# s22s/erased-cells

Hardware: AMD Instinct MI355X
Metric: Gcells/s + HBM-GB/s roofline %, u8/u16->f64 16384^2, 1/2/4/8 GPUs (higher is better)
Workload: dtype f64

## Files before the change

### erased-cells_amd/csrc/ec_abi.hip

```cpp
#include <hip/hip_runtime.h>


#include <cfloat>
#include <cstdarg>
#include <cstdio>
#include <cstring>
#include <map>
#include <mutex>
#include <string>

#include "ec_lattice.hpp"
#include "ec_map_kernels.hpp"
#include "ec_reduce_kernels.hpp"
#include "ec_runtime.hpp"

namespace ecd {

static_assert(kMaxReduceBlocks <= kFinalizeMaxParts, "the finalize kernels read at most kFinalizeMaxParts partials");

static ec_status ensure_init() { return ensure_ready(); }

static int64_t* result_words(const Scratch& sc) { return sc.host_dev ? sc.host_dev : sc.dev_result(); }
static ec_status fetch_result(const Scratch& sc, int words, hipStream_t s) {
    if (!sc.host_dev) {
// ... 12 lines not shown
    }
    return nb < want ? nb : want;
}

static int reduce_cap(int per_cu) {
    const int knob = tuning().reduce_bpc;
    const long cap = long(device_cus()) * (knob > 0 ? knob : per_cu);
    return static_cast<int>(cap < kMaxReduceBlocks ? cap : kMaxReduceBlocks);
}

static inline hipStream_t S(ec_stream s) { return static_cast<hipStream_t>(s); }

template <typename Fn> struct pure_store : std::false_type {};
template <typename W> struct pure_store<FillFn<W>> : std::true_type {};

template <typename Fn, int U>
static void launch_map_u(const Fn& fn, size_t n, hipStream_t s) {
    const size_t groups = n / Fn::CPL;
    const size_t tiles = (groups + size_t(kBlock) * U - 1) / (size_t(kBlock) * U);
    const size_t stream_bytes[2] = {n * Fn::kIn0, n * Fn::kIn1};
    const unsigned lds = (pure_store<Fn>::value ? static_cast<unsigned>(tuning().write_lds_kb.load())
                                                : (Fn::kIn0 != 0 ? static_cast<unsigned>(tuning().map_lds_kb.load()) : 0u)) << 10;
    k_map<Fn, U><<<grid_for(tiles), kBlock, lds, s>>>(fn, n, cache_plan(stream_bytes, 2));
}

template <typename Fn>
static ec_status launch_map(const Fn& fn, size_t n, bool aligned, hipStream_t s, const char* what) {
    if (n == 0) return EC_OK;
    if (!aligned) {
        k_map_cellwise<Fn><<<grid_capped((n + kBlock - 1) / kBlock, 8), kBlock, 0, s>>>(fn, n);
    } else {
        switch (tuning().map_u) {
            case 1: launch_map_u<Fn, 1>(fn, n, s); break;
            case 4: launch_map_u<Fn, 4>(fn, n, s); break;
            default: launch_map_u<Fn, 2>(fn, n, s); break;
        }
    }
    return check_launch(what);
// ... 43 lines not shown
        const bool al = aligned16(p, p, p) && (!mask || aligned_to(mask, 16 / sizeof(T)));
        const int cap = reduce_cap(8);
        if (al) {
            const unsigned head = reduce_head(p, sizeof(T), n);
            const size_t groups = (n - head) / (16 / sizeof(T));
            auto launch = [&](auto u_tag, auto block_tag, int per_cu) {
                constexpr int U = decltype(u_tag)::value, BLOCK = decltype(block_tag)::value;
                static const int resident[2] = {resident_per_cu(k_min_max_partials<T, false, U, BLOCK>, BLOCK, per_cu),
                                                resident_per_cu(k_min_max_partials<T, true, U, BLOCK>, BLOCK, per_cu)};
                const int cap2 = reduce_cap(resident[mask ? 1 : 0]);
                size_t tiles = (groups + size_t(BLOCK) * U - 1) / (size_t(BLOCK) * U);
                if (tiles < 1) tiles = 1;
                grid = static_cast<unsigned>(tiles < size_t(cap2) ? tiles : size_t(cap2));
                int64_t* direct = grid == 1 ? keys2_dev : nullptr;
                const size_t stream_bytes[2] = {n * sizeof(T), mask ? n : 0};
                const unsigned hp = head | (cache_plan(stream_bytes, 2) << 8);
                if (mask) k_min_max_partials<T, true, U, BLOCK><<<grid, BLOCK, 0, s>>>(tp, mask, n, sc.dev, hp, direct);
                else k_min_max_partials<T, false, U, BLOCK><<<grid, BLOCK, 0, s>>>(tp, nullptr, n, sc.dev, hp, direct);
                return direct != nullptr;
            };
            using std::integral_constant;
            bool direct = false;
            switch (tuning().reduce_shape) {
                case 1: direct = launch(integral_constant<int, 16>{}, integral_constant<int, 512>{}, 4); break;
                case 2: direct = launch(integral_constant<int, 8>{}, integral_constant<int, 256>{}, 8); break;
                case 3: direct = launch(integral_constant<int, 8>{}, integral_constant<int, 1024>{}, 2); break;
                case 4: direct = launch(integral_constant<int, 4>{}, integral_constant<int, 512>{}, 4); break;
                default: direct = launch(integral_constant<int, kReduceU>{}, integral_constant<int, kRBlock>{}, 4); break;
            }
            if (direct) return check_launch("min_max(single workgroup)");
        } else {
// ... 244 lines not shown
    if (st != EC_OK) return st;
    st = fetch_result(sc, 2, S(stream));
    if (st != EC_OK) return st;
    return ec_min_max_decode(t, sc.host, mn, mx);
}

template <typename W>
static ec_status first_diff_w(const void* l, const void* r, size_t n, const Scratch& sc, hipStream_t s, unsigned* grid_out) {
    const int cap = reduce_cap(4);
    const bool al = aligned16(l, r, r);
    const unsigned head = al ? reduce_head(l, sizeof(W), n) : 0u;
    size_t tiles = al ? ((n - head) / (16 / sizeof(W)) + size_t(kRBlock) * kReduceU - 1) / (size_t(kRBlock) * kReduceU) : (n + kRBlock - 1) / kRBlock;
    if (tiles < 1) tiles = 1;
    const unsigned grid = static_cast<unsigned>(tiles < size_t(cap) ? tiles : size_t(cap));
    const size_t stream_bytes[2] = {n * sizeof(W), n * sizeof(W)};
    k_first_diff_partials<W, kReduceU><<<grid, kRBlock, 0, s>>>(static_cast<const W*>(l), static_cast<const W*>(r), n,
                                                               reinterpret_cast<uint64_t*>(sc.dev), al, head | (cache_plan(stream_bytes, 2) << 8));
    *grid_out = grid;
    return check_launch("first_diff(partials)");
}

extern "C" ec_status ec_first_difference(ec_dtype t, const void* l, const void* r, size_t n, uint64_t* index, ec_stream stream) {
    EC_REQUIRE_INIT();
    if (!ecl::valid(t)) return set_error(EC_ERR_UNSUPPORTED_TYPE, "ec_first_difference: bad dtype %d", int(t));
    if (!index || (n > 0 && (!l || !r))) return set_error(EC_ERR_ARG, "ec_first_difference: null pointer");
    *index = n;
    if (n == 0) return EC_OK;
    Scratch sc;
    ec_status st = get_scratch(S(stream), &sc);
    if (st != EC_OK) return st;
    std::lock_guard<std::mutex> turn(*sc.mu);
    unsigned grid = 0;
// ... 125 lines not shown
    Scratch sc;
    ec_status st = get_scratch(S(stream), &sc);
    if (st != EC_OK) return st;
    unsigned grid = 0;
    if (n > 0) {
        const int cap = reduce_cap(4);
        const bool al = aligned_to(m, 16);
        const unsigned head = al ? reduce_head(m, 1, n) : 0u;
        size_t tiles = al ? ((n - head) / 16 + size_t(kRBlock) * kReduceU - 1) / (size_t(kRBlock) * kReduceU) : (n + kRBlock - 1) / kRBlock;
        if (tiles < 1) tiles = 1;
        grid = static_cast<unsigned>(tiles < size_t(cap) ? tiles : size_t(cap));
        uint64_t* direct = grid == 1 ? counts2_dev : nullptr;
        const int one = tuning().counts_one_launch.load();
        uint64_t* acc = (!direct && ((one == 1 && n < (size_t(1) << 29)) || (one >= 2 && n < (size_t(1) << 40)))) ? reinterpret_cast<uint64_t*>(sc.dev_acc()) : nullptr;
        const size_t stream_bytes[1] = {n};
        k_mask_count_partials<kReduceU><<<grid, kRBlock, 0, S(stream)>>>(m, n, reinterpret_cast<uint64_t*>(sc.dev), al,
                                                                        head | (cache_plan(stream_bytes, 1) << 8), direct, acc, counts2_dev);
        st = check_launch("mask_counts(partials)");
        if (st != EC_OK || direct || acc) return st;
    }
    k_mask_count_finalize<<<1, kFinalizeBlock, 0, S(stream)>>>(reinterpret_cast<const uint64_t*>(sc.dev), static_cast<int>(grid), n, counts2_dev);
    return check_launch("mask_counts(finalize)");
}

extern "C" ec_status ec_mask_counts(const uint8_t* m, size_t n, uint64_t* n_true, uint64_t* n_false, ec_stream stream) {
    EC_REQUIRE_INIT();
    if (!n_true || !n_false) return set_error(EC_ERR_ARG, "ec_mask_counts: null pointer");
    Scratch sc;
    ec_status st = get_scratch(S(stream), &sc);
    if (st != EC_OK) return st;
    std::lock_guard<std::mutex> turn(*sc.mu);
    st = ec_mask_counts_device(m, n, reinterpret_cast<uint64_t*>(result_words(sc)), stream);
// ... 38 lines not shown
```

### erased-cells_amd/csrc/ec_binop_tu.hpp

```cpp
#pragma once

#include <hip/hip_runtime.h>

#include <cmath>

#include "ec_binop_kernels.hpp"
#include "ec_runtime.hpp"

namespace ecd {

static inline unsigned lds_cap(int knob, int rule_kb) { return static_cast<unsigned>(knob >= 0 ? knob : rule_kb) << 10; }

template <typename L, typename R, int OP>
static ec_status launch_binop_pair(const void* l, const void* r, size_t n, double* out, hipStream_t s) {
    const Tuning& tu = tuning();
    const L* lp = static_cast<const L*>(l);
    const R* rp = static_cast<const R*>(r);
    constexpr int U = kBinopU;
    if (!aligned16(l, r, out)) {
        k_binop_cellwise<L, R, OP><<<grid_capped((n + kBlock - 1) / kBlock, 8), kBlock, 0, s>>>(lp, rp, out, n);
        return check_launch("binop(cellwise)");
    }
    constexpr bool kCanStage = Staged<L>::value || Staged<R>::value;
    const int variant = tu.binop_variant.load();
    const size_t stream_bytes[2] = {n * sizeof(L), l == r ? 0 : n * sizeof(R)};
    unsigned policy = cache_plan(stream_bytes, 2, n * sizeof(double));
    if (l == r && (policy & 1u)) policy |= 2u;
    constexpr bool kRulePair = kCanStage && ((sizeof(L) == 8) != (sizeof(R) == 8)) && (sizeof(L) <= 4 || sizeof(R) <= 4);
    const bool by_rule = variant < 0 && kRulePair && policy == 0 && n >= (size_t(1) << 20);
    if (kCanStage && (variant == 1 || by_rule)) {
        const size_t tiles = (n / kLdsWaveCells + kWavesPerBlock - 1) / kWavesPerBlock;
        constexpr unsigned kStatic = kWavesPerBlock * unsigned(Staged<L>::kSlabBytes + Staged<R>::kSlabBytes);
        const int knob = tu.binop_lds_kb.load();
        const unsigned lds = knob >= 0 ? unsigned(knob) << 10 : by_rule ? 32000u - kStatic : 0u;
        k_binop_lds<L, R, OP, kNtStore, kNtLoad><<<grid_for(tiles), kBlock, lds, s>>>(lp, rp, out, n);
        if (by_rule) lds_rule_launches().fetch_add(1, std::memory_order_relaxed);
        return check_launch(by_rule ? "binop(lds, by rule)" : "binop(lds)");
    }
    const LoadedStream st[2] = {{l, sizeof(L)}, {r, sizeof(R)}};
    const unsigned head = peel_head(st, 2, n);
    const size_t tiles = (((n - head) >> 1) + size_t(kBlock) * U - 1) / (size_t(kBlock) * U);
    k_binop_direct<L, R, OP, U, kNtStore, kNtLoad><<<grid_for(tiles), kBlock, lds_cap(tuning().binop_lds_kb.load(), sizeof(L) == 8 && sizeof(R) == 8 ? 48 : 0), s>>>(lp, rp, out, n, head | (policy << 8));
    return check_launch("binop(direct)");
}
// ... 7 lines not shown
    constexpr int U = kBinopU;
    if (!aligned16(l, r, out) || !aligned16(lm, rm, om)) {
        k_masked_binop_cellwise<L, R, OP><<<grid_capped((n + kBlock - 1) / kBlock, 8), kBlock, 0, s>>>(lp, lm, rp, rm, out, om, n);
        return check_launch("masked_binop(cellwise)");
    }
    constexpr bool kCanStage = Staged<L>::value || Staged<R>::value;
    if (kCanStage && tu.binop_variant == 1) {
        const size_t tiles = (n / kLdsWaveCells + kWavesPerBlock - 1) / kWavesPerBlock;
        k_masked_binop<L, R, OP, U, kNtStore, kNtLoad, true><<<grid_for(tiles), kBlock, lds_cap(tu.binop_lds_kb.load(), 0), s>>>(lp, lm, rp, rm, out, om, n, 0u);
        return check_launch("masked_binop(lds)");
    }
    const LoadedStream st[2] = {{l, sizeof(L)}, {r, sizeof(R)}};
    const unsigned head = peel_head(st, 2, n);
    const size_t tiles = (((n - head) >> 1) + size_t(kBlock) * U - 1) / (size_t(kBlock) * U);
    const size_t stream_bytes[4] = {n * sizeof(L), l == r ? 0 : n * sizeof(R), n, lm == rm ? 0 : n};
    unsigned policy = cache_plan(stream_bytes, 4, n * sizeof(double));
    if (l == r && (policy & 1u)) policy |= 2u;
    if (lm == rm && (policy & 4u)) policy |= 8u;
    k_masked_binop<L, R, OP, U, kNtStore, kNtLoad, false><<<grid_for(tiles), kBlock, 0, s>>>(lp, lm, rp, rm, out, om, n, head | (policy << 8));
    return check_launch("masked_binop(direct)");
}


template <typename L, int OP>
static ec_status launch_scalar(const void* l, double rhs, size_t n, double* out, hipStream_t s) {
    const L* lp = static_cast<const L*>(l);
    constexpr int U = kBinopU;
    if (!aligned16(l, out, out)) {
        k_binop_scalar_cellwise<L, OP><<<grid_capped((n + kBlock - 1) / kBlock, 8), kBlock, 0, s>>>(lp, rhs, out, n);
        return check_launch("binop_scalar(cellwise)");
    }
    const LoadedStream st[1] = {{l, sizeof(L)}};
    const unsigned head = peel_head(st, 1, n);
    const size_t tiles = (((n - head) >> 1) + size_t(kBlock) * U - 1) / (size_t(kBlock) * U);
    const size_t stream_bytes[1] = {n * sizeof(L)};
    const unsigned policy = cache_plan(stream_bytes, 1, n * sizeof(double));
    const unsigned lds = lds_cap(tuning().scalar_lds_kb.load(), sizeof(L) == 8 ? 32 : 0);
    if constexpr (!is_fp<L>::value) {
        if (std::isfinite(rhs) && !(OP == EC_DIV && rhs == 0.0)) {
            k_binop_scalar_direct<L, OP, U, kNtStore, kNtLoad, false><<<grid_for(tiles), kBlock, lds, s>>>(lp, rhs, out, n, head | (policy << 8));
            return check_launch("binop_scalar(direct, no NaN possible)");
        }
    }
    k_binop_scalar_direct<L, OP, U, kNtStore, kNtLoad><<<grid_for(tiles), kBlock, lds, s>>>(lp, rhs, out, n, head | (policy << 8));
    return check_launch("binop_scalar(direct)");
}

template <int OP>
ec_status dispatch_binop(int lt, const void* l, int rt, const void* r, size_t n, double* out, hipStream_t s) {
#define EC_ROW(LID, LT)                                                                         \
    case LID:                                                                                   \
// ... 60 lines not shown
```

### erased-cells_amd/csrc/ec_expr.hip

```cpp
#include <hip/hip_runtime.h>

#include <atomic>
#include <cstdlib>
#include <cstring>

#include <limits>
#include <mutex>
#include <string>

#include "ec_expr.hpp"
#include "ec_expr_fixed.hpp"
#include "ec_expr_jit.hpp"
#include "ec_lattice.hpp"
#include "ec_runtime.hpp"

using namespace ecd;

static std::atomic<int64_t> g_interpreted{0};

namespace ecd {
int64_t expr_stat(const char* key, bool* known) {
    if (!std::strcmp(key, "expr_interp_launches")) {
        *known = true;
        return g_interpreted.load(std::memory_order_relaxed);
// ... 42 lines not shown
        for (int j = k + 1; j < n_steps && !read_later; ++j) {
            const int me = kRefReg0 + st.dst;
            if (j > k + 1 && (steps[j].a == me || steps[j].b == me)) read_later = true;
            if (steps[j].dst == st.dst) break;
        }
        if (!read_later) w |= kStepNoFile;
        ea.prog[k >> 2] |= w << (16 * (k & 3));
    }
    ea.nstreams = static_cast<int8_t>(n_streams);
    ea.nsteps = static_cast<int8_t>(n_steps);
    return EC_OK;
}

static ec_status prepare_expr(ExprArgs& ea, bool* aligned_out, int* cls, const ec_dtype* dt, const void* const* p, int32_t n_streams,
                              const uint8_t* const* masks, const ec_value* scalars, int32_t n_scalars, const ec_expr_step* steps,
                              int32_t n_steps, size_t n, const char* what) {
    ec_status pst = program_of(ea, dt, n_streams, n_scalars, steps, n_steps, what);
    if (pst != EC_OK) return pst;
    if (!p || (n_scalars > 0 && !scalars)) return set_error(EC_ERR_ARG, "%s: null pointer", what);
    bool aligned = true;
    LoadedStream st[kExprMaxStreams];
    for (int k = 0; k < n_streams; ++k) {
        if (!p[k]) return set_error(EC_ERR_ARG, "%s: stream %d is null", what, k);
        ea.p[k] = p[k];
        aligned = aligned && aligned_to(p[k], 16);
        st[k] = {p[k], ecl::size_of(dt[k])};
        for (int j = 0; j < k && st[k].same_as < 0; ++j)
            if (p[j] == p[k]) st[k].same_as = j;
        cls[k] = fused_class_index(st[k].size);
    }
    for (int k = n_streams; k < kExprMaxStreams; ++k) ea.p[k] = p[0];
    for (int k = 0; k < n_scalars; ++k) {
        if (!ecl::valid(scalars[k].dtype)) return set_error(EC_ERR_ARG, "%s: bad dtype of scalar %d", what, k);
        ea.sc[k] = ec_value_to_f64(&scalars[k]);
    }
    if (masks)
        for (int k = 0; k < n_streams; ++k) {
            const ec_status mst = add_mask(masks[k], k, what, ea.m, &ea.nmask, &aligned);
            if (mst != EC_OK) return mst;
        }
    *aligned_out = aligned;
    ea.head = static_cast<uint8_t>(peel_head(st, n_streams, n));
    ea.cacheable = static_cast<uint8_t>(stream_policy(st, ea.nmask, n));
    return EC_OK;
}

static ec_status launch_expr(const ec_dtype* dt, const void* const* p, int32_t n_streams, const uint8_t* const* masks,
                             const ec_value* scalars, int32_t n_scalars, const ec_expr_step* steps, int32_t n_steps, size_t n,
                             double* out, uint8_t* out_mask, hipStream_t s, const char* what) {
    ExprArgs ea{};
    bool aligned = true;
    int cls[kExprMaxStreams] = {0, 0, 0, 0};
    if (!out) return set_error(EC_ERR_ARG, "%s: null pointer", what);
    if (masks && !out_mask) return set_error(EC_ERR_ARG, "%s: null out_mask", what);
    ec_status pst = prepare_expr(ea, &aligned, cls, dt, p, n_streams, masks, scalars, n_scalars, steps, n_steps, n, what);
    if (pst != EC_OK) return pst;
    aligned = aligned && aligned_to(out, 16) && (!masks || aligned_to(out_mask, 16));
    if (!aligned) {
        ea.head = 0;
        k_expr_cellwise<0><<<grid_capped((n + kBlock - 1) / kBlock, 8), kBlock, 0, s>>>(ea, out, out_mask, n);
        return check_launch("expr(cellwise)");
    }
    bool fixed = false;
    ec_status fst = expr_fixed_launch(ea, n, out, out_mask, s, &fixed);
    if (fst != EC_OK) return fst;
    if (fixed) return check_launch("expr(ahead-of-time)");
    bool compiled = false;
    ec_status jst = expr_jit_launch(ea, n, out, out_mask, nullptr, s, &compiled);
    if (jst != EC_OK) return jst;
    if (compiled) return check_launch("expr(compiled)");
// ... 32 lines not shown

static ec_status expr_min_max_keys(const ec_dtype* dt, const void* const* p, const uint8_t* const* masks_or_null, int32_t n_streams,
                                   const ec_value* scalars, int32_t n_scalars, const ec_expr_step* steps, int32_t n_steps, size_t n,
                                   int64_t* keys2_dev, hipStream_t s, const char* what) {
    ec_status st;
    {
        ExprArgs probe{};
        if ((st = program_of(probe, dt, n_streams, n_scalars, steps, n_steps, what)) != EC_OK) return st;
    }
    if (!keys2_dev) return set_error(EC_ERR_ARG, "%s: null keys", what);
    if ((st = check_hip(hipMemcpyAsync(keys2_dev, kF64Identities, sizeof kF64Identities, hipMemcpyHostToDevice, s), "hipMemcpyAsync(keys)")) != EC_OK) return st;
    if (n == 0) return EC_OK;
    ExprArgs ea{};
    bool aligned = true;
    int cls[kExprMaxStreams] = {0, 0, 0, 0};
    if ((st = prepare_expr(ea, &aligned, cls, dt, p, n_streams, masks_or_null, scalars, n_scalars, steps, n_steps, n, what)) != EC_OK) return st;
    if (aligned) {
        bool compiled = false;
        if ((st = expr_jit_launch(ea, n, nullptr, nullptr, keys2_dev, s, &compiled)) != EC_OK) return st;
        if (compiled) return EC_OK;
    }
    void *tmp = nullptr, *tmask = nullptr;
    if ((st = ec_alloc_async(&tmp, n * sizeof(double), s)) != EC_OK) return st;
    if (masks_or_null && (st = ec_alloc_async(&tmask, n, s)) != EC_OK) {
        (void)ec_free_async(tmp, s);
        return st;
    }
    st = launch_expr(dt, p, n_streams, masks_or_null, scalars, n_scalars, steps, n_steps, n, static_cast<double*>(tmp), static_cast<uint8_t*>(tmask), s, what);
    if (st == EC_OK) st = ec_min_max_keys(EC_F64, tmp, static_cast<const uint8_t*>(tmask), n, keys2_dev, s);
    const std::string keep = st != EC_OK ? last_error_text() : std::string();
    (void)ec_free_async(tmp, s);
    if (tmask) (void)ec_free_async(tmask, s);
    return st != EC_OK ? set_error_text(st, keep) : EC_OK;
}

extern "C" ec_status ec_expr_min_max_keys(const ec_dtype* dt, const void* const* p, const uint8_t* const* masks_or_null, int32_t n_streams,
                                          const ec_value* scalars, int32_t n_scalars, const ec_expr_step* steps, int32_t n_steps, size_t n,
                                          int64_t* keys2_dev, ec_stream stream) {
    ec_status st = ensure_ready();
    if (st != EC_OK) return st;
    return expr_min_max_keys(dt, p, masks_or_null, n_streams, scalars, n_scalars, steps, n_steps, n, keys2_dev, static_cast<hipStream_t>(stream),
                             "ec_expr_min_max_keys");
}
// ... 52 lines not shown
```

### erased-cells_amd/csrc/ec_fused.hip

```cpp
#include <hip/hip_runtime.h>

#include "ec_fused_any.hpp"
#include "ec_lattice.hpp"

using namespace ecd;

static ec_status launch_fused_any(FusedArgs& fa, int nops, size_t n, double* out, uint8_t* out_mask, hipStream_t s) {
    LoadedStream st[4];
    int cls[4];
    bool small = fa.o2 == EC_DIV && (fa.o1 == EC_ADD || fa.o1 == EC_SUB) && (fa.o3 == EC_ADD || fa.o3 == EC_SUB || fa.o3 == kOpNone);
    for (int k = 0; k < 4; ++k) {
        if (k < nops && !fa.is_sc[k] && fa.alias[k] == k) st[k] = {fa.p[k], ecl::size_of(fa.dt[k])};
        cls[k] = fused_class_index(st[k].size);
        if (k < nops) small = small && !fa.is_sc[k] && ecl::is_integral(fa.dt[k]) && ecl::size_of(fa.dt[k]) <= 2;
    }
    fa.small = small ? 1 : 0;
    fa.head = static_cast<uint8_t>(peel_head(st, 4, n));
    fa.cacheable = static_cast<uint8_t>(stream_policy(st, fa.nmask, n));
    FusedAnyKernel kern = nullptr;
    switch (cls[0]) {
        case 0: kern = fused_any_kernel<0>(cls[1], cls[2], cls[3]); break;
        case 1: kern = fused_any_kernel<1>(cls[1], cls[2], cls[3]); break;
        case 2: kern = fused_any_kernel<2>(cls[1], cls[2], cls[3]); break;
        case 3: kern = fused_any_kernel<4>(cls[1], cls[2], cls[3]); break;
        default: kern = fused_any_kernel<8>(cls[1], cls[2], cls[3]); break;
    }
    if (!kern) return set_error(EC_ERR_ARG, "ec_fused: no kernel for load classes %d %d %d %d", cls[0], cls[1], cls[2], cls[3]);
    launch_stream_tile<kFusedU>(kern, fa.head, n, s, fa, out, out_mask, n);
    return check_launch("fused(any)");
}

static ec_status launch_fused(int o1, int o2, int o3, const ec_dtype dt[4], const void* const p[4],
                              const uint8_t* const masks[4], const ec_value* scalars, size_t n, double* out,
// ... 89 lines not shown
```

### erased-cells_amd/csrc/ec_runtime.hip

```cpp
#include <hip/hip_runtime.h>

#include <atomic>
#include <cstdarg>
#include <cstdint>
#include <cstdio>
#include <cstdlib>
#include <cstring>
#include <map>
#include <memory>
#include <mutex>
#include <string>

#include "ec_hostpipe.hpp"
#include "ec_runtime.hpp"

namespace ecd {

static thread_local std::string t_err;
static thread_local int t_narrow_src = -1, t_narrow_dst = -1;

ec_status set_error(ec_status code, const char* fmt, ...) {
    char buf[512];
    va_list ap;
    va_start(ap, fmt);
// ... 105 lines not shown
    {"expr_fixed", &g_tuning.expr_fixed, nullptr, 0, 1, Out::Bool},
    {"write_lds_kb", &g_tuning.write_lds_kb, nullptr, 0, 64, Out::Clamp},
    {"binop_lds_kb", &g_tuning.binop_lds_kb, nullptr, -1, 64, Out::Clamp},
    {"scalar_lds_kb", &g_tuning.scalar_lds_kb, nullptr, -1, 64, Out::Clamp},
    {"map_lds_kb", &g_tuning.map_lds_kb, nullptr, 0, 64, Out::Clamp},
    {"fused_lds_kb", &g_tuning.fused_lds_kb, nullptr, 0, 64, Out::Clamp},
    {"counts_one_launch", &g_tuning.counts_one_launch, nullptr, 0, 2, Out::Clamp},
    {"cache_force", &g_tuning.cache_force, nullptr, -1, 255, Out::Refuse},
    {"pool_keep_mb", nullptr, &g_tuning.pool_keep_mb, 0, kMaxMiB, Out::Clamp},
};
const Knob* knob_of(const char* key) {
    for (const Knob& k : kKnobs)
        if (!std::strcmp(k.key, key)) return &k;
    return nullptr;
}
}

int device_cus() { return t_cus; }
int current_device() { return t_active; }


ec_status ensure_ready() {
    if (t_generation != g_generation.load(std::memory_order_acquire)) {
        t_device = -1;
        t_active = -1;
        t_generation = g_generation.load(std::memory_order_acquire);
    }
    const int dev = t_device >= 0 ? t_device : g_default_device.load(std::memory_order_acquire);
    if (dev < 0) return set_error(EC_ERR_NOT_INITIALIZED, "ec_init() has not been called (no HIP device bound)");
    int cur = -1;
// ... 129 lines not shown
    int before = -1;
    const bool had = !g_devs.empty() && hipGetDevice(&before) == hipSuccess;
    if (!g_devs.empty()) expr_jit_release();
    for (auto& kv : g_devs) {
        if (hipSetDevice(kv.first) != hipSuccess) continue;
        (void)hipDeviceSynchronize();
        kv.second.scratch.clear();
        if (kv.second.pool) {
            (void)hipMemPoolTrimTo(kv.second.pool, 0);
            (void)hipMemPoolDestroy(kv.second.pool);
        }
    }
    if (had) (void)hipSetDevice(before);
    (void)hipGetLastError();
    g_devs.clear();
    g_default_device.store(-1);
    g_generation.fetch_add(1);
    t_device = t_active = -1;
    return EC_OK;
}

extern "C" const char* ec_last_error_string(void) { return t_err.c_str(); }

extern "C" ec_status ec_last_narrowing(ec_dtype* src, ec_dtype* dst) {
    if (!src || !dst || t_narrow_src < 0) return set_error(EC_ERR_ARG, "ec_last_narrowing: nothing recorded");
    *src = static_cast<ec_dtype>(t_narrow_src);
    *dst = static_cast<ec_dtype>(t_narrow_dst);
    return EC_OK;
}

// ... 137 lines not shown
    }
    return EC_OK;
}

extern "C" ec_status ec_stream_destroy(ec_stream s) {
    ec_status st = ec_release_stream(s);
    if (st != EC_OK) return st;
    return check_hip(hipStreamDestroy(S(s)), "hipStreamDestroy");
}
extern "C" ec_status ec_stream_sync(ec_stream s) { return check_hip(hipStreamSynchronize(S(s)), "hipStreamSynchronize"); }

extern "C" ec_status ec_stat_get(const char* key, int64_t* value) {
    if (!key || !value) return set_error(EC_ERR_ARG, "ec_stat_get: null argument");
    if (!std::strcmp(key, "pool_allocs")) *value = g_pool_allocs.load(std::memory_order_relaxed);
    else if (!std::strcmp(key, "binop_lds_rule_launches")) *value = g_lds_rule_launches.load(std::memory_order_relaxed);
    else if (!std::strncmp(key, "tune.", 5)) {
        const Knob* kn = knob_of(key + 5);
        if (!kn) return set_error(EC_ERR_ARG, "ec_stat_get: unknown knob '%s'", key + 5);
        *value = kn->i ? int64_t(kn->i->load()) : kn->l->load();
    } else if (!std::strcmp(key, "devices")) {
        std::lock_guard<std::mutex> lk(g_mu);
        *value = static_cast<int64_t>(g_devs.size());
    } else if (!std::strcmp(key, "scratch_streams")) {
        std::lock_guard<std::mutex> lk(g_mu);
        int64_t n = 0;
        for (auto& kv : g_devs) n += static_cast<int64_t>(kv.second.scratch.size());
        *value = n;
    } else {
        bool known = false;
        *value = expr_stat(key, &known);
// ... 26 lines not shown
```

### erased-cells_amd/csrc/ec_runtime.hpp

```cpp
#pragma once

#include <hip/hip_runtime.h>
#include <stddef.h>
#include <stdint.h>

#include <atomic>
#include <memory>
#include <mutex>
#include <string>

#include "erased_cells.h"

namespace ecd {

constexpr int kBinopU = 2;
#ifndef EC_NT_STORE
#define EC_NT_STORE 1
#endif
#ifndef EC_NT_LOAD
#define EC_NT_LOAD 1
#endif
constexpr bool kNtStore = EC_NT_STORE;
constexpr bool kNtLoad = EC_NT_LOAD;
constexpr int kReduceU = 8;
constexpr int kMaxReduceBlocks = 4096;
// ... 50 lines not shown
struct LoadedStream {
    const void* p = nullptr;
    size_t size = 0;
    int same_as = -1;
};
inline unsigned peel_head(const LoadedStream* st, int count, size_t n) {
    if (n < 2 || !tuning().peel) return 0;
    unsigned c0 = 0, c1 = 0;
    for (int k = 0; k < count; ++k) {
        c0 += peel_cost(st[k].p, st[k].size, 0);
        c1 += peel_cost(st[k].p, st[k].size, 1);
    }
    return c1 < c0 ? 1u : 0u;
}

inline unsigned cache_plan(const size_t* bytes, int n, size_t value_out_bytes = 0) {
    const int forced = tuning().cache_force.load();
    if (forced >= 0) return static_cast<unsigned>(forced) & ((1u << (n < 8 ? n : 8)) - 1u);
    const size_t budget = static_cast<size_t>(tuning().mall_mb.load()) << 20;
    unsigned plan = 0;
    size_t used = 0, largest_taken = 0;
    bool taken[8] = {false, false, false, false, false, false, false, false};
    for (int round = 0; round < n && n <= 8; ++round) {
        int best = -1;
        for (int k = 0; k < n; ++k)
            if (!taken[k] && bytes[k] > 0 && (best < 0 || bytes[k] < bytes[best])) best = k;
        if (best < 0 || used + bytes[best] > budget) break;
        taken[best] = true;
        used += bytes[best];
        if (bytes[best] > largest_taken) largest_taken = bytes[best];
        plan |= 1u << best;
    }
    if (value_out_bytes > 0 && plan != 0)
        for (int k = 0; k < n && n <= 8; ++k)
            if (!taken[k] && bytes[k] > 0 && bytes[k] <= largest_taken) return 0;
    return plan;
}

inline unsigned stream_policy(const LoadedStream (&st)[4], int nmask, size_t n) {
    size_t bytes[8] = {0, 0, 0, 0, 0, 0, 0, 0};
    for (int k = 0; k < 4; ++k) bytes[k] = st[k].same_as < 0 ? n * st[k].size : 0;
    for (int j = 0; j < nmask; ++j) bytes[4 + j] = n;
    unsigned policy = cache_plan(bytes, 8, n * sizeof(double));
    for (int k = 0; k < 4; ++k)
        if (st[k].same_as >= 0) policy = (policy & ~(1u << k)) | (((policy >> st[k].same_as) & 1u) << k);
    return policy;
}

inline ec_status add_mask(const uint8_t* m, int k, const char* what, const uint8_t** ms, int8_t* nmask, bool* aligned) {
    if (!m) return set_error(EC_ERR_ARG, "%s: null mask %d", what, k);
    for (int j = 0; j < *nmask; ++j)
        if (ms[j] == m) return EC_OK;
    ms[(*nmask)++] = m;
    *aligned = *aligned && aligned_to(m, 16);
    return EC_OK;
}

inline unsigned reduce_head(const void* p, size_t cell_size, size_t n) {
// ... 37 lines not shown
```

### erased-cells_amd/csrc/ec_window.hip

```cpp
#include <hip/hip_runtime.h>

#include "ec_lattice.hpp"
#include "ec_runtime.hpp"
#include "ec_window_kernels.hpp"

namespace ecd {

static bool mul_overflows(uint64_t a, uint64_t b) { return a != 0 && b > UINT64_MAX / a; }

static ec_status check_window(const char* what, ec_dtype t, uint64_t cols, uint64_t rows, uint64_t x0, uint64_t y0, uint64_t w, uint64_t h,
                              const void* mask_a, const void* mask_b) {
    if (!ecl::valid(t)) return set_error(EC_ERR_UNSUPPORTED_TYPE, "%s: bad dtype %d", what, int(t));
    if (mul_overflows(cols, rows))
        return set_error(EC_ERR_ARG, "%s: a raster of %llu x %llu cells overflows 64 bits", what, (unsigned long long)cols, (unsigned long long)rows);
    if (x0 > cols || w > cols - x0 || y0 > rows || h > rows - y0)
        return set_error(EC_ERR_ARG, "%s: the window (%llu, %llu) + %llu x %llu leaves the raster of %llu x %llu cells", what, (unsigned long long)x0,
                         (unsigned long long)y0, (unsigned long long)w, (unsigned long long)h, (unsigned long long)cols, (unsigned long long)rows);
    if ((mask_a == nullptr) != (mask_b == nullptr)) return set_error(EC_ERR_ARG, "%s: one mask without the other", what);
    return EC_OK;
}

static bool make_axis(uint64_t win, uint64_t out, WindowAxis* a) {
    a->q = win / out;
    a->r = win % out;
// ... 3 lines not shown
    if (worst > UINT64_MAX) return false;
    const uint64_t num = a->q * out + a->r;
    a->d0 = num / (2 * out);
    a->rem0 = num % (2 * out);
    return true;
}

static bool rows_aligned(const void* raster, const WindowGeom& g, size_t cell, const void* contiguous) {
    return ((reinterpret_cast<uintptr_t>(raster) + g.origin * cell) | (g.pitch * cell) | (g.w * cell) | reinterpret_cast<uintptr_t>(contiguous)) % 16 == 0;
}

template <int W, bool MASKED>
static ec_status launch_window(int kind, const WindowArgs& args, const WindowAxis* ax, const WindowAxis* ay, bool vector, hipStream_t s) {
    WindowArgs a = args;
    const size_t bytes[2] = {a.g.n * W, MASKED ? a.g.n : 0};
    a.cacheable = cache_plan(bytes, 2);
    if (!vector) {
        const uint64_t chunks = ((a.g.w + kBlock - 1) / kBlock) * (a.g.n / a.g.w);
        const WindowAxis id_x{1, 0, a.g.w, 0, a.g.w}, id_y{1, 0, a.g.n / a.g.w, 0, a.g.n / a.g.w};
        if (kind == kWinPut) k_window_cellwise<W, MASKED, true><<<grid_capped(chunks, 8), kBlock, 0, s>>>(a, id_x, id_y);
        else k_window_cellwise<W, MASKED, false><<<grid_capped(chunks, 8), kBlock, 0, s>>>(a, ax ? *ax : id_x, ay ? *ay : id_y);
        return check_launch("window(cell-wise)");
    }
    const uint64_t slots = (a.g.n + (16 / W) - 1) / (16 / W), per_tile = uint64_t(kBlock) * kWindowU;
    const unsigned grid = grid_for((slots + per_tile - 1) / per_tile);
    if (uint64_t(grid) * per_tile < slots) return set_error(EC_ERR_ARG, "window: more than 2^31 tiles");
    if (ax) k_window_nearest<W, MASKED><<<grid, kBlock, 0, s>>>(a, *ax, *ay);
    else if (kind == kWinPut) k_window_put<W, MASKED><<<grid, kBlock, 0, s>>>(a);
    else k_window_copy<W, MASKED><<<grid, kBlock, 0, s>>>(a);
    return check_launch(ax ? "window(nearest)" : kind == kWinPut ? "window(put)" : "window(copy)");
}
// ... 59 lines not shown
```

Baseline: 600.7.

## Gate cache-friendly loads on per-device evidence of buffer reuse

Adds a per-device admission ledger that tracks which input buffers were recently read and whether they were read again within a window of twice the MALL budget. Inputs are only marked cacheable (instead of non-temporal) when reuse was seen, or while no losing streak has built up; writes that overlap a tracked buffer invalidate its entry. The aim is to stop polluting the last-level cache with streaming inputs that are never reused. The cost is host-side locking and a ledger lookup on every launch, and a change in cache hints for kernels whose inputs are reused.

```diff
diff --git a/erased-cells_amd/csrc/ec_abi.hip b/erased-cells_amd/csrc/ec_abi.hip
--- a/erased-cells_amd/csrc/ec_abi.hip
+++ b/erased-cells_amd/csrc/ec_abi.hip
@@ -50,6 +50,19 @@
 template <typename Fn> struct pure_store : std::false_type {};
 template <typename W> struct pure_store<FillFn<W>> : std::true_type {};
 
+struct MapStreams {
+    const void* in[2];
+    const void* out;
+    size_t out_cell;
+};
+template <typename S_, typename D_> static MapStreams streams_of(const ConvertFn<S_, D_>& f) { return {{f.src, nullptr}, f.dst, sizeof(D_)}; }
+template <typename T> static MapStreams streams_of(const NegFn<T>& f) { return {{f.src, nullptr}, f.dst, sizeof(typename NegFn<T>::O)}; }
+template <typename W> static MapStreams streams_of(const MaskFromNodataFn<W>& f) { return {{f.src, nullptr}, f.mask, 1}; }
+template <typename W> static MapStreams streams_of(const MaskSelectFn<W>& f) { return {{f.src, f.mask}, f.dst, sizeof(W)}; }
+template <int KIND> static MapStreams streams_of(const MaskBin<KIND>& f) { return {{f.l, f.r}, f.out, 1}; }
+static MapStreams streams_of(const MaskNot& f) { return {{f.m, nullptr}, f.out, 1}; }
+template <typename Fn> static MapStreams streams_of(const Fn& f) { return {{nullptr, nullptr}, f.dst, Fn::kIn0 == 0 ? 16 / Fn::CPL : 0}; }
+
 template <typename Fn, int U>
 static void launch_map_u(const Fn& fn, size_t n, hipStream_t s) {
     const size_t groups = n / Fn::CPL;
@@ -57,7 +70,9 @@
     const size_t stream_bytes[2] = {n * Fn::kIn0, n * Fn::kIn1};
     const unsigned lds = (pure_store<Fn>::value ? static_cast<unsigned>(tuning().write_lds_kb.load())
                                                 : (Fn::kIn0 != 0 ? static_cast<unsigned>(tuning().map_lds_kb.load()) : 0u)) << 10;
-    k_map<Fn, U><<<grid_for(tiles), kBlock, lds, s>>>(fn, n, cache_plan(stream_bytes, 2));
+    const MapStreams ms = streams_of(fn);
+    const size_t written_bytes[1] = {n * ms.out_cell};
+    k_map<Fn, U><<<grid_for(tiles), kBlock, lds, s>>>(fn, n, cache_plan(ms.in, stream_bytes, 2, s, 0, &ms.out, written_bytes, 1));
 }
 
 template <typename Fn>
@@ -131,7 +146,8 @@
                 grid = static_cast<unsigned>(tiles < size_t(cap2) ? tiles : size_t(cap2));
                 int64_t* direct = grid == 1 ? keys2_dev : nullptr;
                 const size_t stream_bytes[2] = {n * sizeof(T), mask ? n : 0};
-                const unsigned hp = head | (cache_plan(stream_bytes, 2) << 8);
+                const void* const stream_ptrs[2] = {p, mask};
+                const unsigned hp = head | (cache_plan(stream_ptrs, stream_bytes, 2, s) << 8);
                 if (mask) k_min_max_partials<T, true, U, BLOCK><<<grid, BLOCK, 0, s>>>(tp, mask, n, sc.dev, hp, direct);
                 else k_min_max_partials<T, false, U, BLOCK><<<grid, BLOCK, 0, s>>>(tp, nullptr, n, sc.dev, hp, direct);
                 return direct != nullptr;
@@ -406,8 +422,9 @@
     if (tiles < 1) tiles = 1;
     const unsigned grid = static_cast<unsigned>(tiles < size_t(cap) ? tiles : size_t(cap));
     const size_t stream_bytes[2] = {n * sizeof(W), n * sizeof(W)};
+    const void* const stream_ptrs[2] = {l, r};
     k_first_diff_partials<W, kReduceU><<<grid, kRBlock, 0, s>>>(static_cast<const W*>(l), static_cast<const W*>(r), n,
-                                                               reinterpret_cast<uint64_t*>(sc.dev), al, head | (cache_plan(stream_bytes, 2) << 8));
+                                                               reinterpret_cast<uint64_t*>(sc.dev), al, head | (cache_plan(stream_ptrs, stream_bytes, 2, s) << 8));
     *grid_out = grid;
     return check_launch("first_diff(partials)");
 }
@@ -563,8 +580,9 @@
         const int one = tuning().counts_one_launch.load();
         uint64_t* acc = (!direct && ((one == 1 && n < (size_t(1) << 29)) || (one >= 2 && n < (size_t(1) << 40)))) ? reinterpret_cast<uint64_t*>(sc.dev_acc()) : nullptr;
         const size_t stream_bytes[1] = {n};
+        const void* const stream_ptrs[1] = {m};
         k_mask_count_partials<kReduceU><<<grid, kRBlock, 0, S(stream)>>>(m, n, reinterpret_cast<uint64_t*>(sc.dev), al,
-                                                                        head | (cache_plan(stream_bytes, 1) << 8), direct, acc, counts2_dev);
+                                                                        head | (cache_plan(stream_ptrs, stream_bytes, 1, S(stream)) << 8), direct, acc, counts2_dev);
         st = check_launch("mask_counts(partials)");
         if (st != EC_OK || direct || acc) return st;
     }
diff --git a/erased-cells_amd/csrc/ec_admission.hpp b/erased-cells_amd/csrc/ec_admission.hpp
--- /dev/null
+++ b/erased-cells_amd/csrc/ec_admission.hpp
@@ -0,0 +1,111 @@
+#pragma once
+
+#include <stddef.h>
+#include <stdint.h>
+
+namespace ecd {
+
+constexpr int kLedgerEntries = 32;
+constexpr uint64_t kWindowBudgets = 2;
+constexpr int kLosingStreak = 4;
+
+struct AdmissionStats {
+    int64_t bets = 0;
+    int64_t won = 0;
+    int64_t lost = 0;
+    int64_t nt_launches = 0;
+    int64_t live = 0;
+};
+
+struct AdmissionLedger {
+    struct Entry {
+        uintptr_t p = 0;
+        size_t bytes = 0;
+        uint64_t clock = 0;
+        bool cacheable = false;
+    };
+    Entry e[kLedgerEntries];
+    uint64_t clock = 0;
+    int streak = 0;
+    AdmissionStats stats;
+
+    void lose(Entry& x, bool counts) {
+        if (x.cacheable) {
+            ++stats.lost;
+            --stats.live;
+            if (counts && streak < kLosingStreak) ++streak;
+        }
+        x = Entry();
+    }
+
+    unsigned decide(const void* const* p, const size_t* bytes, int n, unsigned candidates, const void* const* wp, const size_t* wbytes,
+                    int nw, uint64_t window, bool update) {
+        if (update)
+            for (Entry& x : e)
+                if (x.p && clock - x.clock > window) lose(x, true);
+        unsigned plan = 0, touched = 0;
+        bool denied = false;
+        uint64_t after = clock;
+        for (int k = 0; k < n; ++k) after += bytes[k];
+        for (int j = 0; j < nw; ++j) after += wbytes[j];
+        for (int k = 0; k < n && k < 32; ++k) {
+            if (!((candidates >> k) & 1u) || bytes[k] == 0 || !p[k]) continue;
+            const uintptr_t key = reinterpret_cast<uintptr_t>(p[k]);
+            int at = -1;
+            for (int i = 0; i < kLedgerEntries; ++i)
+                if (e[i].p == key && (e[i].clock >= clock || clock - e[i].clock <= window)) { at = i; break; }
+            if (at >= 0) {
+                plan |= 1u << k;
+                if (!update || ((touched >> at) & 1u)) continue;
+                if (e[at].cacheable) {
+                    ++stats.won;
+                    streak = 0;
+                } else {
+                    ++stats.live;
+                }
+                ++stats.bets;
+                e[at].cacheable = true;
+                e[at].bytes = bytes[k];
+                e[at].clock = after;
+                touched |= 1u << at;
+                continue;
+            }
+            const bool admit = streak < kLosingStreak;
+            if (admit) plan |= 1u << k;
+            else denied = true;
+            if (!update) continue;
+            int slot = -1;
+            for (int i = 0; i < kLedgerEntries && slot < 0; ++i)
+                if (!e[i].p) slot = i;
+            if (slot < 0) {
+                for (int i = 0; i < kLedgerEntries; ++i) {
+                    if ((touched >> i) & 1u) continue;
+                    if (slot < 0 || (e[i].cacheable != e[slot].cacheable ? !e[i].cacheable : e[i].clock < e[slot].clock)) slot = i;
+                }
+                if (slot < 0) continue;
+                lose(e[slot], false);
+            }
+            e[slot].p = key;
+            e[slot].bytes = bytes[k];
+            e[slot].clock = after;
+            e[slot].cacheable = admit;
+            touched |= 1u << slot;
+            if (admit) {
+                ++stats.bets;
+                ++stats.live;
+            }
+        }
+        if (!update) return plan;
+        if (denied) ++stats.nt_launches;
+        for (int j = 0; j < nw; ++j) {
+            if (!wp[j] || !wbytes[j]) continue;
+            const uintptr_t lo = reinterpret_cast<uintptr_t>(wp[j]), hi = lo + wbytes[j];
+            for (Entry& x : e)
+                if (x.p && x.p < hi && lo < x.p + x.bytes) lose(x, true);
+        }
+        clock = after;
+        return plan;
+    }
+};
+
+}
diff --git a/erased-cells_amd/csrc/ec_binop_tu.hpp b/erased-cells_amd/csrc/ec_binop_tu.hpp
--- a/erased-cells_amd/csrc/ec_binop_tu.hpp
+++ b/erased-cells_amd/csrc/ec_binop_tu.hpp
@@ -24,10 +24,14 @@
     constexpr bool kCanStage = Staged<L>::value || Staged<R>::value;
     const int variant = tu.binop_variant.load();
     const size_t stream_bytes[2] = {n * sizeof(L), l == r ? 0 : n * sizeof(R)};
-    unsigned policy = cache_plan(stream_bytes, 2, n * sizeof(double));
+    const void* const stream_ptrs[2] = {l, r};
+    const void* const written[1] = {out};
+    const size_t written_bytes[1] = {n * sizeof(double)};
+    unsigned candidates = 0;
+    unsigned policy = cache_plan(stream_ptrs, stream_bytes, 2, s, n * sizeof(double), written, written_bytes, 1, &candidates);
     if (l == r && (policy & 1u)) policy |= 2u;
     constexpr bool kRulePair = kCanStage && ((sizeof(L) == 8) != (sizeof(R) == 8)) && (sizeof(L) <= 4 || sizeof(R) <= 4);
-    const bool by_rule = variant < 0 && kRulePair && policy == 0 && n >= (size_t(1) << 20);
+    const bool by_rule = variant < 0 && kRulePair && candidates == 0 && n >= (size_t(1) << 20);
     if (kCanStage && (variant == 1 || by_rule)) {
         const size_t tiles = (n / kLdsWaveCells + kWavesPerBlock - 1) / kWavesPerBlock;
         constexpr unsigned kStatic = kWavesPerBlock * unsigned(Staged<L>::kSlabBytes + Staged<R>::kSlabBytes);
@@ -65,7 +69,10 @@
     const unsigned head = peel_head(st, 2, n);
     const size_t tiles = (((n - head) >> 1) + size_t(kBlock) * U - 1) / (size_t(kBlock) * U);
     const size_t stream_bytes[4] = {n * sizeof(L), l == r ? 0 : n * sizeof(R), n, lm == rm ? 0 : n};
-    unsigned policy = cache_plan(stream_bytes, 4, n * sizeof(double));
+    const void* const stream_ptrs[4] = {l, r, lm, rm};
+    const void* const written[2] = {out, om};
+    const size_t written_bytes[2] = {n * sizeof(double), n};
+    unsigned policy = cache_plan(stream_ptrs, stream_bytes, 4, s, n * sizeof(double), written, written_bytes, 2);
     if (l == r && (policy & 1u)) policy |= 2u;
     if (lm == rm && (policy & 4u)) policy |= 8u;
     k_masked_binop<L, R, OP, U, kNtStore, kNtLoad, false><<<grid_for(tiles), kBlock, 0, s>>>(lp, lm, rp, rm, out, om, n, head | (policy << 8));
@@ -85,7 +92,10 @@
     const unsigned head = peel_head(st, 1, n);
     const size_t tiles = (((n - head) >> 1) + size_t(kBlock) * U - 1) / (size_t(kBlock) * U);
     const size_t stream_bytes[1] = {n * sizeof(L)};
-    const unsigned policy = cache_plan(stream_bytes, 1, n * sizeof(double));
+    const void* const stream_ptrs[1] = {l};
+    const void* const written[1] = {out};
+    const size_t written_bytes[1] = {n * sizeof(double)};
+    const unsigned policy = cache_plan(stream_ptrs, stream_bytes, 1, s, n * sizeof(double), written, written_bytes, 1);
     const unsigned lds = lds_cap(tuning().scalar_lds_kb.load(), sizeof(L) == 8 ? 32 : 0);
     if constexpr (!is_fp<L>::value) {
         if (std::isfinite(rhs) && !(OP == EC_DIV && rhs == 0.0)) {
diff --git a/erased-cells_amd/csrc/ec_expr.hip b/erased-cells_amd/csrc/ec_expr.hip
--- a/erased-cells_amd/csrc/ec_expr.hip
+++ b/erased-cells_amd/csrc/ec_expr.hip
@@ -80,7 +80,8 @@
 
 static ec_status prepare_expr(ExprArgs& ea, bool* aligned_out, int* cls, const ec_dtype* dt, const void* const* p, int32_t n_streams,
                               const uint8_t* const* masks, const ec_value* scalars, int32_t n_scalars, const ec_expr_step* steps,
-                              int32_t n_steps, size_t n, const char* what) {
+                              int32_t n_steps, size_t n, const char* what, const void* out, const void* out_mask, hipStream_t s,
+                              int policy_known = -1) {
     ec_status pst = program_of(ea, dt, n_streams, n_scalars, steps, n_steps, what);
     if (pst != EC_OK) return pst;
     if (!p || (n_scalars > 0 && !scalars)) return set_error(EC_ERR_ARG, "%s: null pointer", what);
@@ -107,19 +108,19 @@
         }
     *aligned_out = aligned;
     ea.head = static_cast<uint8_t>(peel_head(st, n_streams, n));
-    ea.cacheable = static_cast<uint8_t>(stream_policy(st, ea.nmask, n));
+    ea.cacheable = static_cast<uint8_t>(policy_known >= 0 ? unsigned(policy_known) : stream_policy(st, ea.m, ea.nmask, n, out, out_mask, s));
     return EC_OK;
 }
 
 static ec_status launch_expr(const ec_dtype* dt, const void* const* p, int32_t n_streams, const uint8_t* const* masks,
                              const ec_value* scalars, int32_t n_scalars, const ec_expr_step* steps, int32_t n_steps, size_t n,
-                             double* out, uint8_t* out_mask, hipStream_t s, const char* what) {
+                             double* out, uint8_t* out_mask, hipStream_t s, const char* what, int policy_known = -1) {
     ExprArgs ea{};
     bool aligned = true;
     int cls[kExprMaxStreams] = {0, 0, 0, 0};
     if (!out) return set_error(EC_ERR_ARG, "%s: null pointer", what);
     if (masks && !out_mask) return set_error(EC_ERR_ARG, "%s: null out_mask", what);
-    ec_status pst = prepare_expr(ea, &aligned, cls, dt, p, n_streams, masks, scalars, n_scalars, steps, n_steps, n, what);
+    ec_status pst = prepare_expr(ea, &aligned, cls, dt, p, n_streams, masks, scalars, n_scalars, steps, n_steps, n, what, out, out_mask, s, policy_known);
     if (pst != EC_OK) return pst;
     aligned = aligned && aligned_to(out, 16) && (!masks || aligned_to(out_mask, 16));
     if (!aligned) {
@@ -182,7 +183,7 @@
     ExprArgs ea{};
     bool aligned = true;
     int cls[kExprMaxStreams] = {0, 0, 0, 0};
-    if ((st = prepare_expr(ea, &aligned, cls, dt, p, n_streams, masks_or_null, scalars, n_scalars, steps, n_steps, n, what)) != EC_OK) return st;
+    if ((st = prepare_expr(ea, &aligned, cls, dt, p, n_streams, masks_or_null, scalars, n_scalars, steps, n_steps, n, what, nullptr, nullptr, s)) != EC_OK) return st;
     if (aligned) {
         bool compiled = false;
         if ((st = expr_jit_launch(ea, n, nullptr, nullptr, keys2_dev, s, &compiled)) != EC_OK) return st;
@@ -194,7 +195,7 @@
         (void)ec_free_async(tmp, s);
         return st;
     }
-    st = launch_expr(dt, p, n_streams, masks_or_null, scalars, n_scalars, steps, n_steps, n, static_cast<double*>(tmp), static_cast<uint8_t*>(tmask), s, what);
+    st = launch_expr(dt, p, n_streams, masks_or_null, scalars, n_scalars, steps, n_steps, n, static_cast<double*>(tmp), static_cast<uint8_t*>(tmask), s, what, ea.cacheable);
     if (st == EC_OK) st = ec_min_max_keys(EC_F64, tmp, static_cast<const uint8_t*>(tmask), n, keys2_dev, s);
     const std::string keep = st != EC_OK ? last_error_text() : std::string();
     (void)ec_free_async(tmp, s);
diff --git a/erased-cells_amd/csrc/ec_fused.hip b/erased-cells_amd/csrc/ec_fused.hip
--- a/erased-cells_amd/csrc/ec_fused.hip
+++ b/erased-cells_amd/csrc/ec_fused.hip
@@ -16,7 +16,7 @@
     }
     fa.small = small ? 1 : 0;
     fa.head = static_cast<uint8_t>(peel_head(st, 4, n));
-    fa.cacheable = static_cast<uint8_t>(stream_policy(st, fa.nmask, n));
+    fa.cacheable = static_cast<uint8_t>(stream_policy(st, fa.m, fa.nmask, n, out, out_mask, s));
     FusedAnyKernel kern = nullptr;
     switch (cls[0]) {
         case 0: kern = fused_any_kernel<0>(cls[1], cls[2], cls[3]); break;
diff --git a/erased-cells_amd/csrc/ec_runtime.hip b/erased-cells_amd/csrc/ec_runtime.hip
--- a/erased-cells_amd/csrc/ec_runtime.hip
+++ b/erased-cells_amd/csrc/ec_runtime.hip
@@ -143,6 +143,53 @@
         if (!std::strcmp(k.key, key)) return &k;
     return nullptr;
 }
+}
+
+namespace {
+constexpr int kLedgerDevices = 16;
+struct DeviceLedger {
+    std::mutex mu;
+    AdmissionLedger ledger;
+};
+DeviceLedger g_ledgers[kLedgerDevices];
+}
+
+unsigned admit_by_evidence(const void* const* ptrs, const size_t* bytes, int n, unsigned candidates, const void* const* wp, const size_t* wbytes,
+                           int nw, uint64_t window, hipStream_t s) {
+    const int dev = t_active;
+    if (dev < 0 || dev >= kLedgerDevices) return candidates;
+    hipStreamCaptureStatus capture = hipStreamCaptureStatusNone;
+    if (hipStreamIsCapturing(s, &capture) != hipSuccess) {
+        (void)hipGetLastError();
+        capture = hipStreamCaptureStatusNone;
+    }
+    DeviceLedger& d = g_ledgers[dev];
+    std::lock_guard<std::mutex> lk(d.mu);
+    return d.ledger.decide(ptrs, bytes, n, candidates, wp, wbytes, nw, window, capture == hipStreamCaptureStatusNone);
+}
+
+static bool ledger_stat(const char* key, int64_t* value) {
+    int64_t AdmissionStats::*field = nullptr;
+    if (!std::strcmp(key, "cache_bets")) field = &AdmissionStats::bets;
+    else if (!std::strcmp(key, "cache_bets_won")) field = &AdmissionStats::won;
+    else if (!std::strcmp(key, "cache_bets_lost")) field = &AdmissionStats::lost;
+    else if (!std::strcmp(key, "cache_bets_live")) field = &AdmissionStats::live;
+    else if (!std::strcmp(key, "cache_nt_launches")) field = &AdmissionStats::nt_launches;
+    else if (!std::strcmp(key, "cache_losing_streak")) {
+        const int dev = t_active >= 0 ? t_active : g_default_device.load(std::memory_order_acquire);
+        *value = 0;
+        if (dev >= 0 && dev < kLedgerDevices) {
+            std::lock_guard<std::mutex> lk(g_ledgers[dev].mu);
+            *value = g_ledgers[dev].ledger.streak;
+        }
+        return true;
+    } else return false;
+    *value = 0;
+    for (DeviceLedger& d : g_ledgers) {
+        std::lock_guard<std::mutex> lk(d.mu);
+        *value += d.ledger.stats.*field;
+    }
+    return true;
 }
 
 int device_cus() { return t_cus; }
@@ -302,6 +349,10 @@
     if (had) (void)hipSetDevice(before);
     (void)hipGetLastError();
     g_devs.clear();
+    for (DeviceLedger& d : g_ledgers) {
+        std::lock_guard<std::mutex> ll(d.mu);
+        d.ledger = AdmissionLedger();
+    }
     g_default_device.store(-1);
     g_generation.fetch_add(1);
     t_device = t_active = -1;
@@ -469,6 +520,7 @@
     if (!key || !value) return set_error(EC_ERR_ARG, "ec_stat_get: null argument");
     if (!std::strcmp(key, "pool_allocs")) *value = g_pool_allocs.load(std::memory_order_relaxed);
     else if (!std::strcmp(key, "binop_lds_rule_launches")) *value = g_lds_rule_launches.load(std::memory_order_relaxed);
+    else if (ledger_stat(key, value)) {}
     else if (!std::strncmp(key, "tune.", 5)) {
         const Knob* kn = knob_of(key + 5);
         if (!kn) return set_error(EC_ERR_ARG, "ec_stat_get: unknown knob '%s'", key + 5);
diff --git a/erased-cells_amd/csrc/ec_runtime.hpp b/erased-cells_amd/csrc/ec_runtime.hpp
--- a/erased-cells_amd/csrc/ec_runtime.hpp
+++ b/erased-cells_amd/csrc/ec_runtime.hpp
@@ -9,6 +9,7 @@
 #include <mutex>
 #include <string>
 
+#include "ec_admission.hpp"
 #include "erased_cells.h"
 
 namespace ecd {
@@ -89,10 +90,16 @@
     return c1 < c0 ? 1u : 0u;
 }
 
-inline unsigned cache_plan(const size_t* bytes, int n, size_t value_out_bytes = 0) {
+unsigned admit_by_evidence(const void* const* ptrs, const size_t* bytes, int n, unsigned candidates, const void* const* wp, const size_t* wbytes,
+                           int nw, uint64_t window, hipStream_t s);
+inline unsigned cache_plan(const void* const* ptrs, const size_t* bytes, int n, hipStream_t s, size_t value_out_bytes = 0,
+                           const void* const* wp = nullptr, const size_t* wbytes = nullptr, int nw = 0, unsigned* candidates = nullptr) {
+    unsigned unused;
+    unsigned& plan_out = candidates ? *candidates : unused;
     const int forced = tuning().cache_force.load();
-    if (forced >= 0) return static_cast<unsigned>(forced) & ((1u << (n < 8 ? n : 8)) - 1u);
+    if (forced >= 0) return plan_out = static_cast<unsigned>(forced) & ((1u << (n < 8 ? n : 8)) - 1u);
     const size_t budget = static_cast<size_t>(tuning().mall_mb.load()) << 20;
+    if (budget == 0) return plan_out = 0;
     unsigned plan = 0;
     size_t used = 0, largest_taken = 0;
     bool taken[8] = {false, false, false, false, false, false, false, false};
@@ -108,15 +115,26 @@
     }
     if (value_out_bytes > 0 && plan != 0)
         for (int k = 0; k < n && n <= 8; ++k)
-            if (!taken[k] && bytes[k] > 0 && bytes[k] <= largest_taken) return 0;
-    return plan;
+            if (!taken[k] && bytes[k] > 0 && bytes[k] <= largest_taken) plan = 0;
+    plan_out = plan;
+    return admit_by_evidence(ptrs, bytes, n <= 8 ? n : 0, plan, wp, wbytes, nw, kWindowBudgets * budget, s);
 }
 
-inline unsigned stream_policy(const LoadedStream (&st)[4], int nmask, size_t n) {
+inline unsigned stream_policy(const LoadedStream (&st)[4], const uint8_t* const* ms, int nmask, size_t n, const void* out, const void* out_mask,
+                              hipStream_t s) {
     size_t bytes[8] = {0, 0, 0, 0, 0, 0, 0, 0};
-    for (int k = 0; k < 4; ++k) bytes[k] = st[k].same_as < 0 ? n * st[k].size : 0;
-    for (int j = 0; j < nmask; ++j) bytes[4 + j] = n;
-    unsigned policy = cache_plan(bytes, 8, n * sizeof(double));
+    const void* ptrs[8] = {nullptr, nullptr, nullptr, nullptr, nullptr, nullptr, nullptr, nullptr};
+    for (int k = 0; k < 4; ++k) {
+        bytes[k] = st[k].same_as < 0 ? n * st[k].size : 0;
+        ptrs[k] = st[k].p;
+    }
+    for (int j = 0; j < nmask; ++j) {
+        bytes[4 + j] = n;
+        ptrs[4 + j] = ms[j];
+    }
+    const void* wp[2] = {out, out_mask};
+    const size_t wbytes[2] = {n * sizeof(double), out_mask ? n : 0};
+    unsigned policy = cache_plan(ptrs, bytes, 8, s, n * sizeof(double), wp, wbytes, 2);
     for (int k = 0; k < 4; ++k)
         if (st[k].same_as >= 0) policy = (policy & ~(1u << k)) | (((policy >> st[k].same_as) & 1u) << k);
     return policy;
diff --git a/erased-cells_amd/csrc/ec_window.hip b/erased-cells_amd/csrc/ec_window.hip
--- a/erased-cells_amd/csrc/ec_window.hip
+++ b/erased-cells_amd/csrc/ec_window.hip
@@ -41,7 +41,10 @@
 static ec_status launch_window(int kind, const WindowArgs& args, const WindowAxis* ax, const WindowAxis* ay, bool vector, hipStream_t s) {
     WindowArgs a = args;
     const size_t bytes[2] = {a.g.n * W, MASKED ? a.g.n : 0};
-    a.cacheable = cache_plan(bytes, 2);
+    const size_t in_at = kind == kWinPut ? 0 : a.g.origin, out_at = kind == kWinPut ? a.g.origin : 0;
+    const void* const ptrs[2] = {static_cast<const char*>(a.in) + in_at * W, MASKED ? a.in_mask + in_at : nullptr};
+    const void* const written[2] = {static_cast<const char*>(a.out) + out_at * W, MASKED ? a.out_mask + out_at : nullptr};
+    a.cacheable = cache_plan(ptrs, bytes, 2, s, 0, written, bytes, 2);
     if (!vector) {
         const uint64_t chunks = ((a.g.w + kBlock - 1) / kBlock) * (a.g.n / a.g.w);
         const WindowAxis id_x{1, 0, a.g.w, 0, a.g.w}, id_y{1, 0, a.g.n / a.g.w, 0, a.g.n / a.g.w};
```

Result: no change. 602.1 (median of 3 runs) (+0.2%).
